# arihantb2/direct_lidar_odometry

Hardware: AMD Instinct MI355X
Metric: gicp_iterations_per_sec (higher is better)
Workload: dtype f64

## Files before the change

direct_lidar_odometry_amd/csrc/ngicp_align.h:

```cpp
#pragma once

namespace {

std::mutex& persist_mutex(int device) {
  static std::mutex m[64];
  return m[(unsigned)device % 64u];
}

route::Facts route_facts(const ngicp* h, route::Caller caller, int nblocks = 1) {
  route::Facts f;
  f.caller = caller;
  f.persist = h->persist;
  f.robust = h->robust_kind != NGICP_ROBUST_NONE;
  f.prior = h->prior_set;
  f.iterating = h->p.max_iter > 0;
  f.nblocks = nblocks;
  f.pass_slots = h->pass_slots;
  f.persist_slots = h->persist_slots;
  f.max_passes = max_passes(h->p);
  return f;
}
void refuse_for(const ngicp* h, route::Entry e) {
  const std::string why = route::entry_refusal(e, h->voxel_res > 0.0, h->robust_kind != NGICP_ROBUST_NONE, h->prior_set);
  if (!why.empty()) throw ArgError{NGICP_ERR_ARG, why};
}
void refuse_route(const ngicp* h, route::Caller caller, const char* entry) {
  const std::string why = route::refusal(route::switches(), h->sw, route_facts(h, caller), entry);
  if (!why.empty()) throw ArgError{NGICP_ERR_ARG, why};
}
route::Variant pass_variant(const ngicp* h, route::Caller caller, int nblocks) {
  return route::choose_route(route::switches(), h->sw, route_facts(h, caller, nblocks)).variant;
}
void fill_robust(const ngicp* h, int& kind, double& c, double& c2) {
  kind = h->robust_kind;
  c = h->robust_width;
  c2 = h->robust_width * h->robust_width;
}

void launch_pass(ngicp* h, const PassArgs& a, const route::Variant& v, int nblocks, hipStream_t s, hipEvent_t start = nullptr, hipEvent_t stop = nullptr) {
  using K = void (*)(PassArgs);
  const bool four = v.waves == 4;
  K kernel = nullptr;
  PassArgs b = a;
  unsigned grid = (unsigned)nblocks;
  switch (v.family) {
    case route::Family::Staged: {
      int need = kStGrowMax;
      if (h->p.max_corr_dist < 1e30) need = (int)std::ceil(h->p.max_corr_dist / (double)a.grid.h);
      b.stage_grow = std::max(1, std::min(kStGrowMax, need));
      kernel = four ? K(k_gicp_pass_st<4>) : K(k_gicp_pass_st<3>);
      break;
    }
    case route::Family::Queue:
      grid = (unsigned)std::min(nblocks, h->queue_slots[four]);
      kernel = four ? K(k_gicp_queue<2, 4>) : K(k_gicp_queue<2, 3>);
      break;
    case route::Family::Walks:
      if (v.fused) kernel = four ? K(k_gicp_pass<2, 4, true>) : K(k_gicp_pass<2, 3, true>);
      else if (v.robust) kernel = four ? K(k_gicp_pass<2, 4, false, true>) : K(k_gicp_pass<2, 3, false, true>);
      else kernel = four ? K(k_gicp_pass<2, 4>) : K(k_gicp_pass<2, 3>);
      break;
  }
  hipExtLaunchKernelGGL(kernel, dim3(grid), dim3(256), 0, s, start, stop, 0, b);
}

struct LoopCtx {
  PassArgs pa;
  SolveArgs sa;
  int nblocks;
};

void prepare_loop(ngicp* h, LoopCtx& c, bool own_buffers = true, bool with_target = true) {
  ensure_slot_ready(h, h->src, "source");
  if (with_target) ensure_slot_ready(h, h->tgt, "target");
  if (h->src_covs.n != h->src.dev->n) compute_covs(h, h->src, h->src_covs, "source");
  if (with_target && h->tgt_covs.n != h->tgt.dev->n) compute_covs(h, h->tgt, h->tgt_covs, "target");
  DeviceCloud& S = *h->src.dev;
  const size_t n = S.n;
  const int nblocks = std::max(1, (S.n_batches + 3) / 4);
  const int max_rows = max_trace_rows(h->p);
  if (own_buffers) {
    for (int i = 0; i < 2; ++i) {
      h->tpt[i].ensure(n * sizeof(float4));
      h->mahal[i].ensure(n * 6 * sizeof(double));
    }
    h->partials.ensure((size_t)kNumSlots * nblocks * sizeof(double));
    h->grp_order.ensure((size_t)nblocks * sizeof(int));
    h->grp_order_alt.ensure((size_t)nblocks * sizeof(int));
    h->grp_cost.ensure((size_t)nblocks * sizeof(int));
    {
      const long ring = (long)max_rows + 1;
      h->state.ensure(sizeof(LmState) + (ring <= kMaxPersistPasses ? (size_t)ring * kViewWords * sizeof(int) : 0));
    }
    if (h->trace.ensure_grew((size_t)max_rows * kTraceCols * sizeof(double))) h->trace_rows_dev = 0;
    h->sums.ensure(kPartialStride * sizeof(double));
    h->batch_far.ensure((size_t)S.n_batches + 16);
    h->gen_lines.ensure((size_t)kGenLines * kGenStride * sizeof(int));
  }

  PassArgs& a = c.pa;
  fill_robust(h, a.robust_kind, a.robust_c, a.robust_c2);
  a.qpts = S.qpts.as<float4>();
  a.batches = S.batches.as<int2>();
  a.batch_boxes = S.batch_boxes.as<float>();
  int* const order_buf[2] = {own_buffers ? h->grp_order.as<int>() : nullptr, own_buffers ? h->grp_order_alt.as<int>() : nullptr};
  int* const ctl = own_buffers ? h->order_flag.as<int>() : nullptr;
  int* const order_flag[2] = {ctl, ctl ? ctl + 3 : nullptr};
  a.grp_order = order_buf[h->order_sel];
  a.grp_cost = own_buffers ? h->grp_cost.as<int>() : nullptr;
  a.n_batches = S.n_batches;
  a.cov_src = covs_for(h, h->src_covs, h->src.dev);
  a.n_src = (int)n;
  if (with_target) {
    DeviceCloud& T = *h->tgt.dev;
    a.tgt = T.pts();
    a.tgt3 = T.xyz3();
    a.tgtp = T.xyzp();
    a.tgt_cell_start = T.cells();
    a.tgt_cell_box = (h->sw.cell_boxes && T.has_boxes) ? T.cell_box.as<unsigned int>() + kCellPad : nullptr;
    a.cov_tgt = covs_for(h, h->tgt_covs, h->tgt.dev);
    a.grid = T.grid;
  } else {
    a.tgt = nullptr;
    a.tgt3 = nullptr;
    a.tgtp = nullptr;
    a.tgt_cell_start = nullptr;
    a.tgt_cell_box = nullptr;
    a.cov_tgt = nullptr;
    a.grid = Grid{};
  }
  for (int i = 0; i < 2; ++i) {
    a.tpt[i] = own_buffers ? h->tpt[i].as<float4>() : nullptr;
    a.mahal[i] = own_buffers ? h->mahal[i].as<double>() : nullptr;
  }
  a.gate_sq = h->p.max_corr_dist * h->p.max_corr_dist;
  {
    float f = (float)a.gate_sq;
    if ((double)f < a.gate_sq) f = std::nextafter(f, std::numeric_limits<float>::infinity());
    a.gate_sq_f = f;
  }
  a.batch_far = own_buffers ? h->batch_far.as<unsigned char>() : nullptr;
  a.st = own_buffers ? h->state.as<LmState>() : nullptr;
  a.partials = own_buffers ? h->partials.as<double>() : nullptr;
  a.mode = 3;
  a.dbg_stamps = nullptr;
  a.dbg_qstats = nullptr;
  a.dbg_span = nullptr;
  a.order_valid = order_flag[h->order_sel];
  a.t_first = nullptr;
  a.fused = 0;
  a.persist = 0;
  a.first_pass = 0;
  a.max_passes = 0;
  a.ticket = ctl ? ctl + 1 : nullptr;
  a.gen = own_buffers ? h->gen_lines.as<int>() : nullptr;
  {
    int need = kStageMaxGrow;
    if (with_target && h->p.max_corr_dist < 1e30) need = (int)std::ceil(h->p.max_corr_dist / (double)a.grid.h);
    a.stage_grow = h->sw.stage_grow <= 0 ? 0 : std::max(1, std::min(std::min(kStageMaxGrow, h->sw.stage_grow), need));
  }

  SolveArgs& s = c.sa;
  s.st = a.st;
  s.cfg.max_iterations = h->p.max_iter;
  s.cfg.lm_max_iterations = h->p.lm_max_iter;
  s.cfg.optimizer = h->p.optimizer;
  s.cfg.rot_eps = h->p.rot_eps;
  s.cfg.trans_eps = h->p.trans_eps;
  s.cfg.lm_init_lambda_factor = h->p.lm_init_lambda_factor;
  s.partials = a.partials;
  s.nblocks = nblocks;
  s.grp_order = order_buf[h->order_sel];
  s.grp_cost = a.grp_cost;
  s.trace = own_buffers ? h->trace.as<double>() : nullptr;
  s.max_trace_rows = max_rows;
  s.mode = 0;
  s.sums_out = nullptr;
  s.dbg_stamps = nullptr;
  s.progress_host = nullptr;
  s.final_host = nullptr;
  s.order_valid = order_flag[h->order_sel];
  s.t_first = nullptr;
  s.persist = 0;
  s.pass_honours_word = 0;
  s.serial_step = h->sw.serial_step;
  s.pass_ticks = nullptr;
  s.prior = h->prior_set ? h->prior_dev.as<double>() : nullptr;
  s.st_out = nullptr;
  s.nrows = 0;
  a.crow_in = nullptr;
  a.crow_out = nullptr;
  a.cluster_ticket = nullptr;
  a.done_flag = nullptr;
  c.nblocks = nblocks;
  if (!own_buffers) return;
  h->stats.lanes_per_query = 2;
  h->stats.voxel_size = a.grid.h;
  h->stats.grid_dims[0] = a.grid.nx;
  h->stats.grid_dims[1] = a.grid.ny;
  h->stats.grid_dims[2] = a.grid.nz;
}

void init_state_from_pose(LmState& st, const Pose& x0) {
  std::memset(&st, 0, sizeof(st));
  st.hot.x0 = x0;
  st.hot.xi = x0;
  pose_identity(st.hot.delta);
  for (int r = 0; r < 3; ++r) {
    for (int c = 0; c < 3; ++c) st.xi_f[r * 4 + c] = (float)x0.R[r * 3 + c];
    st.xi_f[r * 4 + 3] = (float)x0.t[r];
  }
  std::memcpy(&st.view[kViewXi], &st.hot.xi, sizeof(Pose));
  std::memcpy(&st.view[kViewXiF], st.xi_f, sizeof(st.xi_f));
  static_assert(sizeof(Pose) == 24 * sizeof(int) && kViewXiF == 24 && sizeof(LmState::xi_f) == 12 * sizeof(int), "LmState::view layout");
  st.hot.lambda = -1.0;
  st.hot.nu = 2.0;
  for (int i = 0; i < 6; ++i) st.hot.final_H[i * 6 + i] = 1.0;
}

template <class F>
Pose pose_from_colmajor(const F m[16]) {
  Pose p;
  for (int r = 0; r < 3; ++r) {
    for (int c = 0; c < 3; ++c) p.R[r * 3 + c] = (double)m[c * 4 + r];
    p.t[r] = (double)m[12 + r];
  }
  return p;
}
void pose_to_colmajor_f(const Pose& p, float m[16]) {
  for (int r = 0; r < 3; ++r) {
    for (int c = 0; c < 3; ++c) m[c * 4 + r] = (float)p.R[r * 3 + c];
    m[12 + r] = (float)p.t[r];
    m[r * 4 + 3] = 0.f;
  }
  m[15] = 1.f;
}

inline void wait_for_the_loop(ngicp* h, unsigned long& spins, double t_loop) {
  if ((++spins & (h->host_wait ? 0xfff : 0xfffff)) == 0 && now_ms() - t_loop > 30000.0) throw ArgError{NGICP_ERR_HIP, "the registration loop did not finish within 30 s"};
  if (h->host_wait) sched_yield(); else __builtin_ia32_pause();
}

void store_result(const LmHot& r, float T[16], int* converged, int* nr_iterations, double* hessian) {
  pose_to_colmajor_f(r.x0, T);
  if (converged) *converged = r.converged;
  if (nr_iterations) *nr_iterations = r.nr_iterations;
  if (hessian)
    for (int rr = 0; rr < 6; ++rr)
      for (int cc = 0; cc < 6; ++cc) hessian[cc * 6 + rr] = r.final_H[rr * 6 + cc];
  if (r.lm_failed) std::fprintf(stderr, "lm not converged!!\n");
}

void publish_alignment(ngicp* h, const LmState& st, float loop_ms, float* aligned, size_t out_stride) {
  store_result(st.hot, h->final_T, &h->converged, &h->nr_iterations, h->final_hessian);
  h->trace_host.clear();
  h->trace_rows_dev = (size_t)st.hot.n_trace;
  if (aligned) download_transformed(h, *h->src.dev, h->final_T, aligned, out_stride);
  if (st.hot.have_lin) h->hook_valid = 2;
  ngicp_stats& s = h->stats;
  s.loop_ms = loop_ms;
  s.passes = st.hot.passes;
  s.outer_iterations = st.hot.nr_iterations + 1;
  s.lm_trials = st.hot.n_trace;
  s.search_passes = st.hot.search_passes;
  s.mean_candidates = st.hot.search_passes > 0 ? st.hot.cand_total / ((double)st.hot.search_passes * (double)h->src.dev->n) : 0.0;
  s.valid_fraction = st.hot.search_passes > 0 ? st.hot.valid_total / ((double)st.hot.search_passes * (double)h->src.dev->n) : 0.0;
  s.pass_ms_total = 0.0;
  s.passes_timed = 0;
}

void sum_event_pass_times(ngicp* h, long passes) {
  if (!h->profiling) return;
  ngicp_stats& s = h->stats;
  const long timed = std::min<long>(passes, (long)h->prof_events.size() / 2);
  int counted = 0;
  for (long i = h->prof_stride / 2; i < timed; i += h->prof_stride) {
    float ms = 0.f;
    if (hipEventElapsedTime(&ms, h->prof_events[2 * i], h->prof_events[2 * i + 1]) == hipSuccess) {
      s.pass_ms_total += ms;
      ++counted;
    }
  }
  s.passes_timed = counted;
}

struct Alignment {
  double t_begin = now_ms(), t_loop = 0.0;
  LmState st;
  float loop_ms = 0.f;
  unsigned long spins = 0;
};

void reset_results(ngicp* h) {
  h->hook_valid = 0;
  h->converged = 0;
  h->nr_iterations = 0;
  std::memcpy(h->final_T, kIdentity16, sizeof(kIdentity16));
}

const LmState& upload_initial_state(ngicp* h, const float guess[16]) {
  LmState& st = h->pin_state[0];
  init_state_from_pose(st, pose_from_colmajor(guess));
  if (h->p.max_iter <= 0) st.hot.done = 1;
  HIP_TRY(hipMemcpyAsync(h->state.p, &st, sizeof(st), hipMemcpyHostToDevice, h->stream));
  return st;
}

void begin_alignment(ngicp* h, Alignment& al, const float guess[16], SolveArgs& sa, unsigned long long*& pass_t_first) {
  al.st = upload_initial_state(h, guess);
  *h->h_progress = 0;
  sa.progress_host = h->h_progress;
  sa.final_host = h->pin_final;
  sa.t_first = h->t_first.as<unsigned long long>();
  pass_t_first = h->t_first.as<unsigned long long>();
  al.t_loop = now_ms();
}

template <class Launch>
void feed_alignment(ngicp* h, Alignment& al, long max_launches, Launch&& launch) {
  if (h->p.max_iter <= 0) {
    HIP_TRY(hipStreamSynchronize(h->stream));
// ... 666 lines not shown
```

direct_lidar_odometry_amd/csrc/ngicp_lm.h:

```cpp
#pragma once
#include <stddef.h>

#include "ngicp_math.h"
#include "ngicp_terms.h"

namespace ngk {

struct LmConfig {
  int max_iterations;
  int lm_max_iterations;
  int optimizer;
  double rot_eps, trans_eps;
  double lm_init_lambda_factor;
};

struct LmHot {
  Pose x0;
  Pose xi;
  Pose delta;
  double H[36];
  double b[6];
  double y0;
  double d[6];
  double lambda, nu;
  double cand_total;
  double valid_total;
  double staged_total;
  int iter;
  int trial;
  int have_lin;
  int cur;
  int done;
  int converged;
  int nr_iterations;
  int lm_failed;
  int n_trace;
  int passes;
  int pending;
  double final_H[36];
  unsigned long long t_first, t_done;
  float lin_f[12];
  int lin_unneeded;
  int search_passes;
};
constexpr int kViewXi = 0;
constexpr int kViewXiF = 24;
constexpr int kViewDone = 36, kViewCur = 37, kViewHaveLin = 38;
struct LmState {
  LmHot hot;
  float xi_f[12];
  alignas(512) int view[128];
};
constexpr int kViewWords = 128;
constexpr int kGenLines = 256, kGenStride = 32;
static_assert(sizeof(LmState) % 512 == 0 && offsetof(LmState, view) % 512 == 0, "ring entries are 512-byte aligned");

struct PassPose {
  double R[9], t[3];
  float Tf[12];
  int have_lin, cur;
};
typedef const LmState __attribute__((address_space(4))) * KernelStatePtr;
template <class S>
__device__ __forceinline__ void load_pose(S st, PassPose& p) {
  p.have_lin = st->hot.have_lin;
  p.cur = st->hot.cur;
#pragma unroll
  for (int i = 0; i < 9; ++i) p.R[i] = st->hot.xi.R[i];
#pragma unroll
  for (int i = 0; i < 3; ++i) p.t[i] = st->hot.xi.t[i];
#pragma unroll
  for (int i = 0; i < 12; ++i) p.Tf[i] = st->xi_f[i];
}

struct SolveArgs {
  LmState* st;
  LmConfig cfg;
  const double* partials;
  int nblocks;
  double* trace;
  int max_trace_rows;
  int mode;
  double* sums_out;
  int* grp_order;
  const int* grp_cost;
  unsigned long long* dbg_stamps;
  int* progress_host;
  LmHot* final_host;
  int* order_valid;
  const unsigned long long* t_first;
  LmState* st_out;
  int nrows;
  int persist;
  int pass_honours_word;
  int serial_step;
  unsigned long long* pass_ticks;
  const double* prior;
};

static_assert(offsetof(SolveArgs, pass_ticks) == offsetof(SolveArgs, pass_honours_word) + 8, "serial_step takes no room of its own");

__host__ __device__ __forceinline__ int tri21(int r, int c) { return r * 6 - (r * (r - 1)) / 2 + (c - r); }

constexpr int kMaxOrderGroups = 4096;
constexpr int kSolveThreads = 512;
constexpr int kSolveRowSubsets = 32;
constexpr int kProgressDone = 1 << 30, kProgressMask = kProgressDone - 1;

__device__ __forceinline__ bool is_converged_dev(const Pose& d, double rot_eps, double trans_eps) {
  double rmax = 0.0, tmax = 0.0;
#pragma unroll
  for (int r = 0; r < 3; ++r) {
#pragma unroll
    for (int c = 0; c < 3; ++c) rmax = fmax(rmax, 1.0 / rot_eps * fabs(d.R[r * 3 + c] - (r == c ? 1.0 : 0.0)));
    tmax = fmax(tmax, 1.0 / trans_eps * fabs(d.t[r]));
  }
  return fmax(rmax, tmax) < 1;
}

__device__ __forceinline__ double lm_gain_den(const double* d, const double* b, const double lambda) {
  double den = 0.0;
#pragma unroll
  for (int i = 0; i < 6; ++i) den += d[i] * (lambda * d[i] - b[i]);
  return den;
}
__device__ __forceinline__ double lm_step_norm2(const double* d) {
  double dn = 0.0;
#pragma unroll
  for (int i = 0; i < 6; ++i) dn += d[i] * d[i];
  return dn;
}
__device__ __forceinline__ double lm_lambda_accepted(const double lambda, const double rho) {
  const double q = 2 * rho - 1;
  return lambda * fmax(1.0 / 3.0, 1 - q * q * q);
}

__device__ __forceinline__ void make_trial(LmHot& L, double lambda_add) {
  double A[36], rhs[6];
#pragma unroll
  for (int i = 0; i < 36; ++i) A[i] = L.H[i];
#pragma unroll
  for (int i = 0; i < 6; ++i) {
    A[i * 6 + i] += lambda_add;
    rhs[i] = -L.b[i];
  }
  ldlt6_solve(A, rhs, L.d);
  pose_identity(L.delta);
  so3_exp_matrix(L.d, L.delta.R);
  L.delta.t[0] = L.d[3];
  L.delta.t[1] = L.d[4];
  L.delta.t[2] = L.d[5];
  pose_mul(L.delta, L.x0, L.xi);
}

__device__ __forceinline__ void set_lin_unneeded(LmHot& L, const LmConfig& cfg) {
  L.lin_unneeded = (is_converged_dev(L.delta, cfg.rot_eps, cfg.trans_eps) || L.iter + 1 >= cfg.max_iterations) ? 1 : 0;
}

__device__ __forceinline__ void adopt_new(LmHot& L, const double* sums) {
#pragma unroll
  for (int r = 0; r < 6; ++r)
#pragma unroll
    for (int c = r; c < 6; ++c) L.H[r * 6 + c] = L.H[c * 6 + r] = sums[tri21(r, c)];
#pragma unroll
  for (int i = 0; i < 6; ++i) L.b[i] = sums[21 + i];
  L.y0 = sums[27];
  L.cur ^= 1;
  L.have_lin = 1;
#pragma unroll
  for (int r = 0; r < 3; ++r) {
#pragma unroll
    for (int c = 0; c < 3; ++c) L.lin_f[r * 4 + c] = (float)L.xi.R[r * 3 + c];
    L.lin_f[r * 4 + 3] = (float)L.xi.t[r];
  }
}

__device__ __forceinline__ bool lm_advance(LmHot& L, const LmConfig& cfg, const double* sums, double* trace, int max_trace_rows) {
  const double yi = sums[28];
  L.passes += 1;
  L.cand_total += sums[29];
  L.valid_total += sums[30];
  L.staged_total += sums[31];

  if (cfg.optimizer == 0) {
    adopt_new(L, sums);
    L.nr_iterations = L.iter;
    make_trial(L, 0.0);
    L.x0 = L.xi;
    L.converged = is_converged_dev(L.delta, cfg.rot_eps, cfg.trans_eps) ? 1 : 0;
    L.iter += 1;
    if (L.converged || L.iter >= cfg.max_iterations) L.done = 1;
    return true;
  }

  if (!L.have_lin) {
    adopt_new(L, sums);
    L.nr_iterations = 0;
    if (L.lambda < 0.0) {
      double m = 0.0;
#pragma unroll
      for (int i = 0; i < 6; ++i) m = fmax(m, fabs(L.H[i * 6 + i]));
      L.lambda = cfg.lm_init_lambda_factor * m;
    }
    L.nu = 2.0;
    L.trial = 0;
    if (cfg.lm_max_iterations <= 0) {
      L.lm_failed = 1;
      L.done = 1;
      return false;
    }
    make_trial(L, L.lambda);
    set_lin_unneeded(L, cfg);
    return false;
  }

  const double den = lm_gain_den(L.d, L.b, L.lambda), dn = lm_step_norm2(L.d);
  const double rho = (L.y0 - yi) / den;
  const bool rejected = rho < 0;
  if (trace && L.n_trace < max_trace_rows) {
    double* row = trace + (size_t)L.n_trace * kTraceCols;
    row[0] = L.iter; row[1] = L.trial; row[2] = L.y0; row[3] = yi;
    row[4] = rho; row[5] = L.lambda; row[6] = sqrt(dn); row[7] = rejected ? 0.0 : 1.0;
    L.n_trace += 1;
  }
  if (rejected) {
    if (is_converged_dev(L.delta, cfg.rot_eps, cfg.trans_eps)) {
      L.converged = 1;
      L.done = 1;
      return false;
    }
    L.lambda = L.nu * L.lambda;
    L.nu = 2 * L.nu;
    L.trial += 1;
    if (L.trial >= cfg.lm_max_iterations) {
      L.lm_failed = 1;
      L.converged = 0;
      L.done = 1;
      return false;
    }
    make_trial(L, L.lambda);
    set_lin_unneeded(L, cfg);
    return false;
  }
  return true;
}

__device__ __forceinline__ void lm_step(LmHot& L, const LmConfig& cfg, const double* sums, double* trace, int max_trace_rows, const bool searched = true) {
  const bool gn = cfg.optimizer == 0;
  L.search_passes += searched ? 1 : 0;
  const bool accepted = lm_advance(L, cfg, sums, trace, max_trace_rows);
  if (accepted) {
#pragma unroll
    for (int i = 0; i < 36; ++i) L.final_H[i] = L.H[i];
    if (!gn) {
      const double rho = (L.y0 - sums[28]) / lm_gain_den(L.d, L.b, L.lambda);
      L.x0 = L.xi;
      L.lambda = lm_lambda_accepted(L.lambda, rho);
      L.converged = is_converged_dev(L.delta, cfg.rot_eps, cfg.trans_eps) ? 1 : 0;
      L.iter += 1;
      if (L.converged || L.iter >= cfg.max_iterations) {
        L.done = 1;
      } else {
        adopt_new(L, sums);
        L.nr_iterations = L.iter;
        L.nu = 2.0;
        L.trial = 0;
        make_trial(L, L.lambda);
        set_lin_unneeded(L, cfg);
      }
    }
  }
  if (gn && !L.done) L.xi = L.x0;
}

__device__ __forceinline__ void wave_sync() {
  __builtin_amdgcn_fence(__ATOMIC_RELEASE, "wavefront");
  __builtin_amdgcn_wave_barrier();
  __builtin_amdgcn_fence(__ATOMIC_ACQUIRE, "wavefront");
}
__device__ __forceinline__ double wave_lane_f64(const double v, const int src_lane) {
  return __hiloint2double(__builtin_amdgcn_readlane(__double2hiint(v), src_lane), __builtin_amdgcn_readlane(__double2loint(v), src_lane));
}
__device__ __forceinline__ double wave_fetch_f64(const double v, const int src_lane) {
  return __hiloint2double(__builtin_amdgcn_ds_bpermute(src_lane << 2, __double2hiint(v)), __builtin_amdgcn_ds_bpermute(src_lane << 2, __double2loint(v)));
}
__device__ __forceinline__ bool wave_agree(const bool b) { return __builtin_amdgcn_readfirstlane(b ? 1 : 0) != 0; }
__device__ __forceinline__ int pose_elem_to_rows(const int e) { return e < 9 ? (e / 3) * 4 + e % 3 : (e - 9) * 4 + 3; }

__device__ __forceinline__ void adopt_new_wave(LmHot& L, const double* sums, const int lane) {
  if (lane < 36) {
    const int i = lane / 6, j = lane - 6 * i;
    L.H[lane] = sums[tri21(min(i, j), max(i, j))];
  }
  if (lane < 6) L.b[lane] = sums[21 + lane];
  if (lane < 12) L.lin_f[pose_elem_to_rows(lane)] = (float)reinterpret_cast<const double*>(&L.xi)[lane];
  if (lane == 0) {
    L.y0 = sums[27];
    L.cur ^= 1;
    L.have_lin = 1;
  }
}

__device__ __forceinline__ void make_trial_wave(LmHot& L, const LmConfig& cfg, const double lambda_add, const bool lin_word, const int iter, const int lane) {
  wave_sync();
  const bool act = lane < 36;
  const int i = act ? lane / 6 : 0, j = act ? lane - 6 * i : 0;
  const int r = max(i, j), c = min(i, j);
  double a = act ? L.H[lane] : 0.0;
  if (act && i == j) a += lambda_add;
  double y[6];
#pragma unroll
  for (int e = 0; e < 6; ++e) y[e] = -L.b[e];
  const bool out_t = lane >= 9;
  const int orow = lane < 12 ? (out_t ? lane - 9 : lane / 3) : 0, ocol = lane < 9 ? lane % 3 : 0;
  double xb[3];
#pragma unroll
  for (int m = 0; m < 3; ++m) xb[m] = out_t ? L.x0.t[m] : L.x0.R[m * 3 + ocol];
  int piv[6];
#pragma unroll
  for (int k = 0; k < 6; ++k) {
    int p = k;
    double best = fabs(wave_lane_f64(a, 7 * k));
#pragma unroll
    for (int q = k + 1; q < 6; ++q) {
      const double v = fabs(wave_lane_f64(a, 7 * q));
      if (v > best) {
        best = v;
        p = q;
      }
    }
    p = __builtin_amdgcn_readfirstlane(p);
    piv[k] = p;
    if (p != k) {
      const int si = i == k ? p : (i == p ? k : i), sj = j == k ? p : (j == p ? k : j);
      a = wave_fetch_f64(a, si * 6 + sj);
    }
    if (k < 5) {
      const double dk = wave_lane_f64(a, 7 * k);
      if (dk != 0.0 && isfinite(dk)) {
        const double scaled = ldlt_scale(a, dk);
        if (act && j == k && i > k) a = scaled;
        const double upd = ldlt_update(wave_fetch_f64(a, r * 6 + c), wave_fetch_f64(a, r * 6 + k), dk, wave_fetch_f64(a, c * 6 + k));
        if (act && i > k && j > k) a = upd;
      }
    }
  }
#pragma unroll
  for (int k = 0; k < 6; ++k)
#pragma unroll
    for (int q = k + 1; q < 6; ++q)
      if (piv[k] == q) {
        const double t = y[k];
        y[k] = y[q];
        y[q] = t;
      }
  double lo[15];
#pragma unroll
  for (int q = 1; q < 6; ++q)
#pragma unroll
    for (int e = 0; e < q; ++e) lo[q * (q - 1) / 2 + e] = wave_lane_f64(a, q * 6 + e);
#pragma unroll
  for (int q = 0; q < 6; ++q)
#pragma unroll
    for (int e = 0; e < q; ++e) y[q] = ldlt_subst(y[q], lo[q * (q - 1) / 2 + e], y[e]);
  {
    double mine = y[0];
#pragma unroll
    for (int q = 1; q < 6; ++q) mine = lane == 7 * q ? y[q] : mine;
    const double dv = ldlt_diag(mine, a);
#pragma unroll
    for (int q = 0; q < 6; ++q) y[q] = wave_lane_f64(dv, 7 * q);
  }
#pragma unroll
  for (int q = 5; q >= 0; --q)
#pragma unroll
    for (int e = q + 1; e < 6; ++e) y[q] = ldlt_subst(y[q], lo[e * (e - 1) / 2 + q], y[e]);
#pragma unroll
  for (int k = 5; k >= 0; --k)
#pragma unroll
    for (int q = k + 1; q < 6; ++q)
      if (piv[k] == q) {
        const double t = y[k];
        y[k] = y[q];
        y[q] = t;
      }
  Pose delta;
  so3_exp_matrix(y, delta.R);
  delta.t[0] = y[3];
  delta.t[1] = y[4];
  delta.t[2] = y[5];
  double ar[3];
#pragma unroll
  for (int m = 0; m < 3; ++m) ar[m] = orow == 0 ? delta.R[m] : (orow == 1 ? delta.R[3 + m] : delta.R[6 + m]);
  const double at = orow == 0 ? delta.t[0] : (orow == 1 ? delta.t[1] : delta.t[2]);
  const double xr = pose_mul_r(ar[0], ar[1], ar[2], xb[0], xb[1], xb[2]), xt = pose_mul_t(ar[0], ar[1], ar[2], xb[0], xb[1], xb[2], at);
  if (lane < 12) reinterpret_cast<double*>(&L.xi)[lane] = out_t ? xt : xr;
  const bool conv = lin_word ? is_converged_dev(delta, cfg.rot_eps, cfg.trans_eps) : false;
  if (lane == 0) {
#pragma unroll
    for (int e = 0; e < 6; ++e) L.d[e] = y[e];
    L.delta = delta;
    if (lin_word) L.lin_unneeded = (conv || iter + 1 >= cfg.max_iterations) ? 1 : 0;
  }
}

__device__ __forceinline__ void lm_step_wave(LmHot& L, const LmConfig& cfg, const double* sums, double* trace, int max_trace_rows, const bool searched, const int lane) {
  const double yi = sums[28];
  int iter = L.iter;
  double lambda = L.lambda;
  const int have_lin = L.have_lin;
  if (lane == 0) {
    L.search_passes += searched ? 1 : 0;
    L.passes += 1;
    L.cand_total += sums[29];
    L.valid_total += sums[30];
    L.staged_total += sums[31];
  }
  const bool gn = cfg.optimizer == 0;
  bool go_on = true;
  if (gn) {
    adopt_new_wave(L, sums, lane);
    lambda = 0.0;
  } else if (!wave_agree(have_lin != 0)) {
    adopt_new_wave(L, sums, lane);
    if (wave_agree(lambda < 0.0)) {
      double m = 0.0;
#pragma unroll
      for (int i = 0; i < 6; ++i) m = fmax(m, fabs(sums[tri21(i, i)]));
      lambda = cfg.lm_init_lambda_factor * m;
    }
    go_on = cfg.lm_max_iterations > 0;
    if (lane == 0) {
      L.nr_iterations = 0;
      L.lambda = lambda;
      L.nu = 2.0;
      L.trial = 0;
      if (!go_on) L.lm_failed = 1, L.done = 1;
    }
  } else {
    double d[6], b[6];
#pragma unroll
    for (int e = 0; e < 6; ++e) d[e] = L.d[e], b[e] = L.b[e];
    const double y0 = L.y0, nu = L.nu;
    const int trial = L.trial, n_trace = L.n_trace;
    const double rho = (y0 - yi) / lm_gain_den(d, b, lambda);
    const bool rejected = wave_agree(rho < 0);
    if (trace && n_trace < max_trace_rows && lane == 0) {
      double* row = trace + (size_t)n_trace * kTraceCols;
      row[0] = iter; row[1] = trial; row[2] = y0; row[3] = yi;
      row[4] = rho; row[5] = lambda; row[6] = sqrt(lm_step_norm2(d)); row[7] = rejected ? 0.0 : 1.0;
      L.n_trace = n_trace + 1;
    }
    const bool conv = wave_agree(is_converged_dev(L.delta, cfg.rot_eps, cfg.trans_eps));
    if (rejected) {
      const bool failed = !conv && trial + 1 >= cfg.lm_max_iterations;
      go_on = !conv && !failed;
      if (!conv) lambda = nu * lambda;
      if (lane == 0) {
        if (conv) {
          L.converged = 1, L.done = 1;
        } else {
          L.lambda = lambda;
          L.nu = 2 * nu;
          L.trial = trial + 1;
          if (failed) L.lm_failed = 1, L.converged = 0, L.done = 1;
        }
      }
    } else {
      if (lane < 36) L.final_H[lane] = L.H[lane];
      if (lane < 12) reinterpret_cast<double*>(&L.x0)[lane] = reinterpret_cast<const double*>(&L.xi)[lane];
      lambda = lm_lambda_accepted(lambda, rho);
      iter += 1;
      go_on = !(conv || iter >= cfg.max_iterations);
      if (lane == 0) {
        L.lambda = lambda;
        L.converged = conv ? 1 : 0;
        L.iter = iter;
        if (!go_on) L.done = 1;
      }
      if (go_on) {
        adopt_new_wave(L, sums, lane);
        if (lane == 0) {
          L.nr_iterations = iter;
          L.nu = 2.0;
          L.trial = 0;
        }
      }
    }
  }
  if (!wave_agree(go_on)) return;
  make_trial_wave(L, cfg, lambda, !gn, iter, lane);
  if (gn) {
    wave_sync();
    if (lane < 12) reinterpret_cast<double*>(&L.x0)[lane] = reinterpret_cast<const double*>(&L.xi)[lane];
    if (lane < 36) L.final_H[lane] = L.H[lane];
    const bool conv = wave_agree(is_converged_dev(L.delta, cfg.rot_eps, cfg.trans_eps));
    if (lane == 0) {
      L.nr_iterations = iter;
      L.converged = conv ? 1 : 0;
      L.iter = iter + 1;
      if (conv || iter + 1 >= cfg.max_iterations) L.done = 1;
    }
  }
}

}
```

direct_lidar_odometry_amd/csrc/ngicp_solve.h:

```cpp
#pragma once
#include "ngicp_lm.h"

namespace ngk {

constexpr int kSolveSubs = kSolveThreads / 16;
#ifndef NGICP_SOLVE_CHUNK
#define NGICP_SOLVE_CHUNK 40
#endif
constexpr int kSolveChunk = NGICP_SOLVE_CHUNK;


template <int THREADS>
struct SolveShared {
  double wsum[32][kPartialStride];
  double sums[kPartialStride];
  int ord_cnt[THREADS / 64 - 1][16], ord_pos[THREADS / 64 - 1][16];
  int ord_cost[kMaxOrderGroups];
  unsigned char ord_cls[kMaxOrderGroups];
  int ord_arrived;
  LmHot L;
};

template <int THREADS>
__device__ __forceinline__ void build_launch_order(const SolveArgs& a, SolveShared<THREADS>& sh, const int lane, const int wave) {
  auto& ord_cnt = sh.ord_cnt;
  auto& ord_pos = sh.ord_pos;
  auto& ord_cost = sh.ord_cost;
  auto& ord_cls = sh.ord_cls;
  int& ord_arrived = sh.ord_arrived;
  const unsigned long long t_ord = a.dbg_stamps ? __builtin_amdgcn_s_memtime() : 0ull;
  constexpr int kSortWaves = THREADS / 64 - 1;
  const int sw = wave - 1;
  auto wsync = [] {
    __builtin_amdgcn_fence(__ATOMIC_RELEASE, "wavefront");
    __builtin_amdgcn_wave_barrier();
    __builtin_amdgcn_fence(__ATOMIC_ACQUIRE, "wavefront");
  };
  auto same_class = [&](int cls, bool valid) -> unsigned long long {
    unsigned long long m = __ballot(valid);
#pragma unroll
    for (int bit = 0; bit < 4; ++bit) {
      const bool one = (cls >> bit) & 1;
      const unsigned long long bb = __ballot(valid && one);
      m &= one ? bb : ~bb;
    }
    return m;
  };
  if (lane < 16) ord_cnt[sw][lane] = 0;
  int mx = 1;
  for (int gi = lane; gi < a.nblocks; gi += 64) mx = max(mx, ord_cost[gi]);
#pragma unroll
  for (int o = 32; o > 0; o >>= 1) mx = max(mx, __shfl_xor(mx, o));
  const float to_class = 16.0f / ((float)mx + 1.0f);
  const unsigned long long lt = (1ull << lane) - 1ull;
  const int slice = ((a.nblocks + kSortWaves * 64 - 1) / (kSortWaves * 64)) * 64;
  const int g_first = sw * slice, g_last = min(g_first + slice, a.nblocks);
  wsync();
  for (int g0 = g_first; g0 < g_last; g0 += 64) {
    const int gi = g0 + lane;
    const bool valid = gi < g_last;
    const int cls = valid ? 15 - min(15, (int)((float)ord_cost[gi] * to_class)) : 0;
    if (valid) ord_cls[gi] = (unsigned char)cls;
    const unsigned long long m = same_class(cls, valid);
    if (valid && (m & lt) == 0) ord_cnt[sw][cls] += __popcll(m);
    wsync();
  }
  __builtin_amdgcn_fence(__ATOMIC_RELEASE, "workgroup");
  if (lane == 0) atomicAdd(&ord_arrived, 1);
  bool met = false;
  for (int spin = 0; spin < (1 << 20); ++spin) {
    if (*reinterpret_cast<volatile int*>(&ord_arrived) >= kSortWaves) {
      met = true;
      break;
    }
    __builtin_amdgcn_s_sleep(2);
  }
  __builtin_amdgcn_fence(__ATOMIC_ACQUIRE, "workgroup");
  if (met) {
    if (lane < 16) {
      int run = 0;
      for (int c = 0; c < lane; ++c)
        for (int w = 0; w < kSortWaves; ++w) run += ord_cnt[w][c];
      for (int w = 0; w < sw; ++w) run += ord_cnt[w][lane];
      ord_pos[sw][lane] = run;
    }
    wsync();
    for (int g0 = g_first; g0 < g_last; g0 += 64) {
      const int gi = g0 + lane;
      const bool valid = gi < g_last;
      const int cls = valid ? ord_cls[gi] : 0;
      const unsigned long long m = same_class(cls, valid);
      const int base = ord_pos[sw][cls];
      if (valid) a.grp_order[base + __popcll(m & lt)] = gi;
      wsync();
      if (valid && (m & lt) == 0) ord_pos[sw][cls] = base + __popcll(m);
      wsync();
    }
    if (sw == 0 && lane == 0 && a.order_valid) *a.order_valid = 1;
  }
  if (a.dbg_stamps && sw == 0 && lane == 0) a.dbg_stamps[7] = __builtin_amdgcn_s_memtime() - t_ord;
}

template <int THREADS, bool AGENT, bool PERSIST = false>
__device__ __forceinline__ void lm_solve_body(const SolveArgs& a, SolveShared<THREADS>& sh) {
  static_assert(!PERSIST || AGENT, "the persistent solver is an agent-scope one");
  constexpr int kSolveThreads = THREADS;
  constexpr int kSolveSubs = 32;
  constexpr int kThreadSubs = THREADS / 16;
  constexpr int kPer = kSolveSubs / kThreadSubs;
  constexpr int kSolveChunk = THREADS >= 512 ? NGICP_SOLVE_CHUNK : 14;
  static_assert(kPer >= 1 && kPer * kThreadSubs == kSolveSubs, "block sizes: 256 or 512 threads");
  auto& wsum = sh.wsum;
  auto& sums = sh.sums;
  auto& ord_cost = sh.ord_cost;
  int& ord_arrived = sh.ord_arrived;
  LmHot& L = sh.L;
  if (threadIdx.x == 0) ord_arrived = 0;
  LmState* st = a.st;
  LmState* sto = a.st_out ? a.st_out : a.st;
#define NG_SSTAMP(k)                                                                 \
  do {                                                                               \
    if (a.dbg_stamps && threadIdx.x == 0) a.dbg_stamps[k] = __builtin_amdgcn_s_memtime(); \
  } while (0)
  const int done_at_entry = PERSIST ? 0 : __hip_atomic_load(&st->hot.done, __ATOMIC_RELAXED, __HIP_MEMORY_SCOPE_WORKGROUP);
  const unsigned long long t_solver_entry = a.dbg_stamps ? __builtin_amdgcn_s_memtime() : 0ull;
  const int lane = threadIdx.x & 63, wave = threadIdx.x >> 6;
  const int vp = threadIdx.x & 15, sb = threadIdx.x >> 4;
  const double2* __restrict__ rows = reinterpret_cast<const double2*>(a.partials) + vp;
  static_assert(sizeof(LmHot) % 4 == 0, "LmHot is copied as dwords");
  constexpr int kHotWords = (int)(sizeof(LmHot) / 4), kHotPerThread = (kHotWords + kSolveThreads - 1) / kSolveThreads;
  constexpr int kCostPerThread = kMaxOrderGroups / kSolveThreads;
  const int passes_at_entry = PERSIST ? __hip_atomic_load(&st->hot.passes, __ATOMIC_RELAXED, __HIP_MEMORY_SCOPE_AGENT) : st->hot.passes;
  const int k4_only_at_entry = (!PERSIST && a.pass_honours_word) ? st->hot.lin_unneeded : 0;
  const bool order_it = a.mode == 0 && a.grp_order && a.nblocks <= kMaxOrderGroups && !k4_only_at_entry && (PERSIST ? passes_at_entry == 2 : (!AGENT || passes_at_entry < 3 || (passes_at_entry & 3) == 3));
  int hv[kHotPerThread];
#pragma unroll
  for (int k = 0; k < kHotPerThread; ++k) {
    const int w = threadIdx.x + k * kSolveThreads;
    if constexpr (PERSIST) hv[k] = w < kHotWords ? __hip_atomic_load(reinterpret_cast<const int*>(&st->hot) + w, __ATOMIC_RELAXED, __HIP_MEMORY_SCOPE_AGENT) : 0;
    else hv[k] = w < kHotWords ? reinterpret_cast<const int*>(&st->hot)[w] : 0;
  }
  const int last_row = (a.nrows ? a.nrows : a.nblocks) - 1, last_grp = a.nblocks - 1;
  auto load_row = [](const double2* q) -> double2 {
    if constexpr (PERSIST) {
      const double* d = reinterpret_cast<const double*>(q);
      return make_double2(__hip_atomic_load(d, __ATOMIC_RELAXED, __HIP_MEMORY_SCOPE_AGENT), __hip_atomic_load(d + 1, __ATOMIC_RELAXED, __HIP_MEMORY_SCOPE_AGENT));
    } else {
      return *q;
    }
  };
  double2 p[kPer * kSolveChunk];
#pragma unroll
  for (int sI = 0; sI < kPer; ++sI)
#pragma unroll
    for (int j = 0; j < kSolveChunk; ++j) {
      const int gi = sb + sI * kThreadSubs + j * kSolveSubs;
      p[sI * kSolveChunk + j] = gi <= last_row ? load_row(rows + (size_t)gi * (kNumSlots / 2)) : make_double2(0.0, 0.0);
    }
  int oc[kCostPerThread];
#pragma unroll
  for (int k = 0; k < kCostPerThread; ++k) {
    const int gi = threadIdx.x + k * kSolveThreads;
    if constexpr (PERSIST) oc[k] = (order_it && gi <= last_grp) ? __hip_atomic_load(a.grp_cost + gi, __ATOMIC_RELAXED, __HIP_MEMORY_SCOPE_AGENT) : 0;
    else oc[k] = (order_it && gi <= last_grp) ? a.grp_cost[gi] : 0;
  }
  double prior_v = 0.0;
  if (a.prior && threadIdx.x < kPriorDoubles) prior_v = a.prior[threadIdx.x];
  if (a.mode == 0 && done_at_entry) return;
  if (a.dbg_stamps && threadIdx.x == 0) a.dbg_stamps[0] = t_solver_entry;
#pragma unroll
  for (int k = 0; k < kHotPerThread; ++k) {
    const int w = threadIdx.x + k * kSolveThreads;
    if (w < kHotWords) reinterpret_cast<int*>(&L)[w] = hv[k];
  }
  if (order_it) {
#pragma unroll
    for (int k = 0; k < kCostPerThread; ++k) {
      const int gi = threadIdx.x + k * kSolveThreads;
      if (gi < a.nblocks) ord_cost[gi] = oc[k];
    }
  }
  {
    double a0[kPer], a1[kPer];
#pragma unroll
    for (int sI = 0; sI < kPer; ++sI) {
      a0[sI] = p[sI * kSolveChunk].x;
      a1[sI] = p[sI * kSolveChunk].y;
#pragma unroll
      for (int j = 1; j < kSolveChunk; ++j) {
        a0[sI] += p[sI * kSolveChunk + j].x;
        a1[sI] += p[sI * kSolveChunk + j].y;
      }
    }
    for (int g0 = kSolveSubs * kSolveChunk; g0 + sb <= last_row; g0 += kSolveSubs * kSolveChunk) {
#pragma unroll
      for (int sI = 0; sI < kPer; ++sI)
#pragma unroll
        for (int j = 0; j < kSolveChunk; ++j) {
          const int gi = g0 + sb + sI * kThreadSubs + j * kSolveSubs;
          p[sI * kSolveChunk + j] = gi <= last_row ? load_row(rows + (size_t)gi * (kNumSlots / 2)) : make_double2(0.0, 0.0);
        }
#pragma unroll
      for (int sI = 0; sI < kPer; ++sI)
#pragma unroll
        for (int j = 0; j < kSolveChunk; ++j) {
          a0[sI] += p[sI * kSolveChunk + j].x;
          a1[sI] += p[sI * kSolveChunk + j].y;
        }
    }
    NG_SSTAMP(1);
#pragma unroll
    for (int sI = 0; sI < kPer; ++sI) {
      wsum[sb + sI * kThreadSubs][2 * vp] = a0[sI];
      wsum[sb + sI * kThreadSubs][2 * vp + 1] = a1[sI];
    }
  }
  __syncthreads();
  if (threadIdx.x < kPartialStride) {
    const int v = threadIdx.x;
    double t = 0.0;
    if (v < kNumSlots)
      for (int sb = 0; sb < kSolveSubs; ++sb) t += wsum[sb][v];
    sums[v] = t;
  }
  __syncthreads();
  NG_SSTAMP(2);
  if (a.sums_out && threadIdx.x < kPartialStride) a.sums_out[threadIdx.x] = sums[threadIdx.x];
  if (a.mode == 3) return;
  if (order_it && wave >= 1) build_launch_order<THREADS>(a, sh, lane, wave);
  if (wave != 0) return;
  if (a.prior) {
    double* const P = &wsum[0][0];
    if (lane < kPriorDoubles) P[lane] = prior_v;
    wave_sync();
    double r[6], theta_sq, jc;
    prior_residual(L.xi, P, r, theta_sq, jc);
    if (lane < 36) P[kPriorDoubles + lane] = prior_jac_elem(lane / 6, lane % 6, r[0], r[1], r[2], theta_sq, jc, L.xi.t[0], L.xi.t[1], L.xi.t[2]);
#pragma unroll
    for (int q = 0; q < 6; ++q)
      if (lane == 36 + q) P[kPriorDoubles + 36 + q] = r[q];
    wave_sync();
    if (lane < kPriorRowSums + 1) sums[lane] += prior_row_elem(lane < kPriorRowSums ? lane : kPriorRowSums - 1, P + kPriorDoubles, P + 12, P + kPriorDoubles + 36);
    wave_sync();
  }
  if (a.mode == 2) {
    if (lane == 0) st->hot.y0 = sums[28];
    return;
  }
  if (a.mode != 1 && !a.serial_step) {
    NG_SSTAMP(3);
    lm_step_wave(L, a.cfg, sums, a.trace, a.max_trace_rows, !(a.pass_honours_word && L.lin_unneeded), lane);
    NG_SSTAMP(4);
    wave_sync();
    NG_SSTAMP(5);
    if (!L.done && lane < 12) {
      const float f = (float)reinterpret_cast<const double*>(&L.xi)[lane];
      if constexpr (PERSIST) __hip_atomic_store(&st->xi_f[pose_elem_to_rows(lane)], f, __ATOMIC_RELAXED, __HIP_MEMORY_SCOPE_AGENT);
      else sto->xi_f[pose_elem_to_rows(lane)] = f;
    }
  } else if (lane == 0) {
    if (a.mode == 1) {
      adopt_new(L, sums);
    } else {
      const LmConfig& cfg = a.cfg;
      NG_SSTAMP(3);
      lm_step(L, cfg, sums, a.trace, a.max_trace_rows, !(a.pass_honours_word && L.lin_unneeded));
      NG_SSTAMP(4);
      NG_SSTAMP(5);
      if (!L.done) {
#pragma unroll
        for (int r = 0; r < 3; ++r) {
#pragma unroll
          for (int c = 0; c < 4; ++c) {
            const float f = (float)(c < 3 ? L.xi.R[r * 3 + c] : L.xi.t[r]);
            if constexpr (PERSIST) __hip_atomic_store(&st->xi_f[r * 4 + c], f, __ATOMIC_RELAXED, __HIP_MEMORY_SCOPE_AGENT);
            else sto->xi_f[r * 4 + c] = f;
          }
        }
      }
    }
  }
  if (a.mode == 0 && lane == 0 && L.done) {
    L.t_done = __builtin_amdgcn_s_memrealtime();
    if (a.t_first) L.t_first = PERSIST ? __hip_atomic_load(a.t_first, __ATOMIC_RELAXED, __HIP_MEMORY_SCOPE_AGENT) : *a.t_first;
  }
  __builtin_amdgcn_fence(__ATOMIC_RELEASE, "wavefront");
  __builtin_amdgcn_wave_barrier();
  __builtin_amdgcn_fence(__ATOMIC_ACQUIRE, "wavefront");
  const bool finished_now = a.mode == 0 && L.done != 0;
  if constexpr (!PERSIST) {
    for (int w = lane; w < (int)(sizeof(LmHot) / 4); w += 64) reinterpret_cast<int*>(&sto->hot)[w] = reinterpret_cast<const int*>(&L)[w];
  }
  if (finished_now && a.final_host) {
    for (int w = lane; w < (int)(sizeof(LmHot) / 4); w += 64)
      __hip_atomic_store(reinterpret_cast<int*>(a.final_host) + w, reinterpret_cast<const int*>(&L)[w], __ATOMIC_RELAXED, __HIP_MEMORY_SCOPE_SYSTEM);
    __threadfence_system();
    __builtin_amdgcn_wave_barrier();
  }
  if (a.mode == 0 && a.progress_host && lane == 0)
    __hip_atomic_store(a.progress_host, (L.passes & kProgressMask) | (L.done ? kProgressDone : 0), __ATOMIC_RELAXED, __HIP_MEMORY_SCOPE_SYSTEM);
  if constexpr (PERSIST) {
    for (int w = lane; w < (int)(sizeof(LmHot) / 4); w += 64)
      __hip_atomic_store(reinterpret_cast<int*>(&st->hot) + w, reinterpret_cast<const int*>(&L)[w], __ATOMIC_RELAXED, __HIP_MEMORY_SCOPE_AGENT);
    int v = 0;
    if (lane < 24) {
      v = reinterpret_cast<const int*>(&L.xi)[lane];
    } else if (lane < 36) {
      const int r = (lane - 24) >> 2, cI = (lane - 24) & 3;
      v = __float_as_int((float)(cI < 3 ? L.xi.R[r * 3 + cI] : L.xi.t[r]));
    } else if (lane == kViewDone) {
      v = L.done;
    } else if (lane == kViewCur) {
      v = L.cur;
    } else if (lane == kViewHaveLin) {
      v = L.have_lin;
    }
    __hip_atomic_store(st->view + (size_t)L.passes * kViewWords + lane, v, __ATOMIC_RELAXED, __HIP_MEMORY_SCOPE_AGENT);
  }
  NG_SSTAMP(6);
#undef NG_SSTAMP
}

__global__ void __launch_bounds__(kSolveThreads) k_lm_solve(SolveArgs a) {
  __shared__ SolveShared<kSolveThreads> sh;
  lm_solve_body<kSolveThreads, false>(a, sh);
}

constexpr int kStepSelftestIn = 132;
constexpr size_t kStepSelftestRecord = sizeof(LmHot) + 18 * sizeof(double);
static_assert(sizeof(LmHot) % 8 == 0, "the trace row behind the image is 8-byte aligned");
__global__ void __launch_bounds__(64) k_step_selftest(const double* __restrict__ in, int n_problems, unsigned char* __restrict__ out) {
  __shared__ LmHot L;
  __shared__ double sums[kPartialStride];
  static_assert(kPartialStride >= 32, "32 reduced sums");
  const int lane = threadIdx.x;
  if ((int)blockIdx.x >= n_problems) return;
  const double* p = in + (size_t)blockIdx.x * kStepSelftestIn;
  LmConfig cfg;
  cfg.max_iterations = (int)p[93];
  cfg.lm_max_iterations = (int)p[94];
  cfg.optimizer = (int)p[95];
  cfg.rot_eps = p[96];
  cfg.trans_eps = p[97];
  cfg.lm_init_lambda_factor = p[98];
  const bool searched = p[131] != 0.0;
  for (int form = 0; form < 2; ++form) {
    unsigned char* rec = out + ((size_t)blockIdx.x * 2 + form) * kStepSelftestRecord;
    double* tail = reinterpret_cast<double*>(rec + sizeof(LmHot));
    __syncthreads();
    for (int w = lane; w < (int)(sizeof(LmHot) / 4); w += 64) reinterpret_cast<int*>(&L)[w] = 0;
    if (lane < 32) sums[lane] = p[99 + lane];
    __syncthreads();
    if (lane < 36) reinterpret_cast<double*>(&L.x0)[lane] = p[lane];
    if (lane < 36) L.H[lane] = p[36 + lane];
    if (lane < 6) L.b[lane] = p[72 + lane], L.d[lane] = p[79 + lane];
    if (lane == 0) {
      L.y0 = p[78];
      L.lambda = p[85];
      L.nu = p[86];
      L.iter = (int)p[87];
      L.trial = (int)p[88];
      L.have_lin = (int)p[89];
      L.cur = (int)p[90];
      L.n_trace = max(0, (int)p[91]);
      L.lin_unneeded = (int)p[92];
    }
    __syncthreads();
    if (form == 0) {
      if (lane == 0) lm_step(L, cfg, sums, tail, 1, searched);
    } else {
      lm_step_wave(L, cfg, sums, tail, 1, searched, lane);
    }
    __syncthreads();
    for (int w = lane; w < (int)(sizeof(LmHot) / 4); w += 64) reinterpret_cast<int*>(rec)[w] = reinterpret_cast<const int*>(&L)[w];
    if (lane < 6) tail[8 + lane] = L.d[lane];
    if (lane == 0) tail[14] = L.done, tail[15] = L.converged, tail[16] = L.lm_failed, tail[17] = L.trial;
  }
}
static_assert(offsetof(LmHot, xi) == offsetof(LmHot, x0) + sizeof(Pose) && offsetof(LmHot, delta) == offsetof(LmHot, xi) + sizeof(Pose), "x0, xi, delta are contiguous");

}
```

Baseline: 21000.

## Cache trial convergence, precompute inverse epsilons, vectorize state copy, relax sync

Stores the reciprocal rotation and translation tolerances in the LM config so the convergence test multiplies instead of divides. It caches the convergence verdict of each trial step in a new LmHot field, so the accept and reject paths reuse it instead of recomputing it. The non-persistent state write-back now uses 16-byte stores, and one block-wide barrier after the sums reduction becomes a wave-level sync. The wave sync is only safe if a single wave reads the reduced sums; otherwise it opens a race.

```diff
diff --git a/direct_lidar_odometry_amd/csrc/ngicp_align.h b/direct_lidar_odometry_amd/csrc/ngicp_align.h
--- a/direct_lidar_odometry_amd/csrc/ngicp_align.h
+++ b/direct_lidar_odometry_amd/csrc/ngicp_align.h
@@ -165,8 +165,7 @@
   s.cfg.max_iterations = h->p.max_iter;
   s.cfg.lm_max_iterations = h->p.lm_max_iter;
   s.cfg.optimizer = h->p.optimizer;
-  s.cfg.rot_eps = h->p.rot_eps;
-  s.cfg.trans_eps = h->p.trans_eps;
+  lm_config_set_eps(s.cfg, h->p.rot_eps, h->p.trans_eps);
   s.cfg.lm_init_lambda_factor = h->p.lm_init_lambda_factor;
   s.partials = a.partials;
   s.nblocks = nblocks;
diff --git a/direct_lidar_odometry_amd/csrc/ngicp_lm.h b/direct_lidar_odometry_amd/csrc/ngicp_lm.h
--- a/direct_lidar_odometry_amd/csrc/ngicp_lm.h
+++ b/direct_lidar_odometry_amd/csrc/ngicp_lm.h
@@ -10,9 +10,13 @@
   int max_iterations;
   int lm_max_iterations;
   int optimizer;
-  double rot_eps, trans_eps;
+  double inv_rot_eps, inv_trans_eps;
   double lm_init_lambda_factor;
 };
+__host__ __device__ __forceinline__ void lm_config_set_eps(LmConfig& c, double rot_eps, double trans_eps) {
+  c.inv_rot_eps = 1.0 / rot_eps;
+  c.inv_trans_eps = 1.0 / trans_eps;
+}
 
 struct LmHot {
   Pose x0;
@@ -37,12 +41,17 @@
   int n_trace;
   int passes;
   int pending;
+  int trial_converged;
   double final_H[36];
   unsigned long long t_first, t_done;
   float lin_f[12];
   int lin_unneeded;
   int search_passes;
 };
+static_assert(offsetof(LmHot, trial_converged) + 4 == offsetof(LmHot, final_H) && sizeof(LmHot) % 8 == 0, "trial_converged fills what was padding: no field moved");
+static_assert(offsetof(LmHot, iter) == 720 && offsetof(LmHot, trial) == 724 && offsetof(LmHot, done) == 736 && offsetof(LmHot, converged) == 740 &&
+              offsetof(LmHot, lm_failed) == 748 && offsetof(LmHot, trial_converged) == 764 && offsetof(LmHot, lin_unneeded) == 1120 && offsetof(LmHot, delta) == 192,
+              "the offsets the step tests read");
 constexpr int kViewXi = 0;
 constexpr int kViewXiF = 24;
 constexpr int kViewDone = 36, kViewCur = 37, kViewHaveLin = 38;
@@ -107,13 +116,13 @@
 constexpr int kSolveRowSubsets = 32;
 constexpr int kProgressDone = 1 << 30, kProgressMask = kProgressDone - 1;
 
-__device__ __forceinline__ bool is_converged_dev(const Pose& d, double rot_eps, double trans_eps) {
+__device__ __forceinline__ bool is_converged_dev(const Pose& d, double inv_rot_eps, double inv_trans_eps) {
   double rmax = 0.0, tmax = 0.0;
 #pragma unroll
   for (int r = 0; r < 3; ++r) {
 #pragma unroll
-    for (int c = 0; c < 3; ++c) rmax = fmax(rmax, 1.0 / rot_eps * fabs(d.R[r * 3 + c] - (r == c ? 1.0 : 0.0)));
-    tmax = fmax(tmax, 1.0 / trans_eps * fabs(d.t[r]));
+    for (int c = 0; c < 3; ++c) rmax = fmax(rmax, inv_rot_eps * fabs(d.R[r * 3 + c] - (r == c ? 1.0 : 0.0)));
+    tmax = fmax(tmax, inv_trans_eps * fabs(d.t[r]));
   }
   return fmax(rmax, tmax) < 1;
 }
@@ -154,7 +163,9 @@
 }
 
 __device__ __forceinline__ void set_lin_unneeded(LmHot& L, const LmConfig& cfg) {
-  L.lin_unneeded = (is_converged_dev(L.delta, cfg.rot_eps, cfg.trans_eps) || L.iter + 1 >= cfg.max_iterations) ? 1 : 0;
+  const bool conv = is_converged_dev(L.delta, cfg.inv_rot_eps, cfg.inv_trans_eps);
+  L.trial_converged = conv ? 1 : 0;
+  L.lin_unneeded = (conv || L.iter + 1 >= cfg.max_iterations) ? 1 : 0;
 }
 
 __device__ __forceinline__ void adopt_new(LmHot& L, const double* sums) {
@@ -187,7 +198,7 @@
     L.nr_iterations = L.iter;
     make_trial(L, 0.0);
     L.x0 = L.xi;
-    L.converged = is_converged_dev(L.delta, cfg.rot_eps, cfg.trans_eps) ? 1 : 0;
+    L.converged = is_converged_dev(L.delta, cfg.inv_rot_eps, cfg.inv_trans_eps) ? 1 : 0;
     L.iter += 1;
     if (L.converged || L.iter >= cfg.max_iterations) L.done = 1;
     return true;
@@ -224,7 +235,7 @@
     L.n_trace += 1;
   }
   if (rejected) {
-    if (is_converged_dev(L.delta, cfg.rot_eps, cfg.trans_eps)) {
+    if (L.trial_converged) {
       L.converged = 1;
       L.done = 1;
       return false;
@@ -256,7 +267,7 @@
       const double rho = (L.y0 - sums[28]) / lm_gain_den(L.d, L.b, L.lambda);
       L.x0 = L.xi;
       L.lambda = lm_lambda_accepted(L.lambda, rho);
-      L.converged = is_converged_dev(L.delta, cfg.rot_eps, cfg.trans_eps) ? 1 : 0;
+      L.converged = L.trial_converged ? 1 : 0;
       L.iter += 1;
       if (L.converged || L.iter >= cfg.max_iterations) {
         L.done = 1;
@@ -395,12 +406,12 @@
   const double at = orow == 0 ? delta.t[0] : (orow == 1 ? delta.t[1] : delta.t[2]);
   const double xr = pose_mul_r(ar[0], ar[1], ar[2], xb[0], xb[1], xb[2]), xt = pose_mul_t(ar[0], ar[1], ar[2], xb[0], xb[1], xb[2], at);
   if (lane < 12) reinterpret_cast<double*>(&L.xi)[lane] = out_t ? xt : xr;
-  const bool conv = lin_word ? is_converged_dev(delta, cfg.rot_eps, cfg.trans_eps) : false;
+  const bool conv = lin_word ? is_converged_dev(delta, cfg.inv_rot_eps, cfg.inv_trans_eps) : false;
   if (lane == 0) {
 #pragma unroll
     for (int e = 0; e < 6; ++e) L.d[e] = y[e];
     L.delta = delta;
-    if (lin_word) L.lin_unneeded = (conv || iter + 1 >= cfg.max_iterations) ? 1 : 0;
+    if (lin_word) L.trial_converged = conv ? 1 : 0, L.lin_unneeded = (conv || iter + 1 >= cfg.max_iterations) ? 1 : 0;
   }
 }
 
@@ -451,7 +462,7 @@
       row[4] = rho; row[5] = lambda; row[6] = sqrt(lm_step_norm2(d)); row[7] = rejected ? 0.0 : 1.0;
       L.n_trace = n_trace + 1;
     }
-    const bool conv = wave_agree(is_converged_dev(L.delta, cfg.rot_eps, cfg.trans_eps));
+    const bool conv = wave_agree(L.trial_converged != 0);
     if (rejected) {
       const bool failed = !conv && trial + 1 >= cfg.lm_max_iterations;
       go_on = !conv && !failed;
@@ -494,7 +505,7 @@
     wave_sync();
     if (lane < 12) reinterpret_cast<double*>(&L.x0)[lane] = reinterpret_cast<const double*>(&L.xi)[lane];
     if (lane < 36) L.final_H[lane] = L.H[lane];
-    const bool conv = wave_agree(is_converged_dev(L.delta, cfg.rot_eps, cfg.trans_eps));
+    const bool conv = wave_agree(is_converged_dev(L.delta, cfg.inv_rot_eps, cfg.inv_trans_eps));
     if (lane == 0) {
       L.nr_iterations = iter;
       L.converged = conv ? 1 : 0;
diff --git a/direct_lidar_odometry_amd/csrc/ngicp_solve.h b/direct_lidar_odometry_amd/csrc/ngicp_solve.h
--- a/direct_lidar_odometry_amd/csrc/ngicp_solve.h
+++ b/direct_lidar_odometry_amd/csrc/ngicp_solve.h
@@ -18,7 +18,7 @@
   int ord_cost[kMaxOrderGroups];
   unsigned char ord_cls[kMaxOrderGroups];
   int ord_arrived;
-  LmHot L;
+  alignas(16) LmHot L;
 };
 
 template <int THREADS>
@@ -223,7 +223,7 @@
       for (int sb = 0; sb < kSolveSubs; ++sb) t += wsum[sb][v];
     sums[v] = t;
   }
-  __syncthreads();
+  wave_sync();
   NG_SSTAMP(2);
   if (a.sums_out && threadIdx.x < kPartialStride) a.sums_out[threadIdx.x] = sums[threadIdx.x];
   if (a.mode == 3) return;
@@ -289,7 +289,10 @@
   __builtin_amdgcn_fence(__ATOMIC_ACQUIRE, "wavefront");
   const bool finished_now = a.mode == 0 && L.done != 0;
   if constexpr (!PERSIST) {
-    for (int w = lane; w < (int)(sizeof(LmHot) / 4); w += 64) reinterpret_cast<int*>(&sto->hot)[w] = reinterpret_cast<const int*>(&L)[w];
+    constexpr int kHot16 = (int)(sizeof(LmHot) / 16);
+    static_assert(sizeof(LmHot) % 16 == 8 && offsetof(LmState, hot) == 0 && alignof(LmState) >= 16, "70 sixteen-byte words and one of eight");
+    for (int w = lane; w < kHot16; w += 64) reinterpret_cast<int4*>(&sto->hot)[w] = reinterpret_cast<const int4*>(&L)[w];
+    if (lane == kHot16 % 64) reinterpret_cast<int2*>(&sto->hot)[2 * kHot16] = reinterpret_cast<const int2*>(&L)[2 * kHot16];
   }
   if (finished_now && a.final_host) {
     for (int w = lane; w < (int)(sizeof(LmHot) / 4); w += 64)
@@ -330,7 +333,7 @@
 constexpr size_t kStepSelftestRecord = sizeof(LmHot) + 18 * sizeof(double);
 static_assert(sizeof(LmHot) % 8 == 0, "the trace row behind the image is 8-byte aligned");
 __global__ void __launch_bounds__(64) k_step_selftest(const double* __restrict__ in, int n_problems, unsigned char* __restrict__ out) {
-  __shared__ LmHot L;
+  __shared__ alignas(16) LmHot L;
   __shared__ double sums[kPartialStride];
   static_assert(kPartialStride >= 32, "32 reduced sums");
   const int lane = threadIdx.x;
@@ -340,8 +343,7 @@
   cfg.max_iterations = (int)p[93];
   cfg.lm_max_iterations = (int)p[94];
   cfg.optimizer = (int)p[95];
-  cfg.rot_eps = p[96];
-  cfg.trans_eps = p[97];
+  lm_config_set_eps(cfg, p[96], p[97]);
   cfg.lm_init_lambda_factor = p[98];
   const bool searched = p[131] != 0.0;
   for (int form = 0; form < 2; ++form) {
@@ -364,6 +366,9 @@
       L.cur = (int)p[90];
       L.n_trace = max(0, (int)p[91]);
       L.lin_unneeded = (int)p[92];
+      Pose delta;
+      for (int e = 0; e < 12; ++e) reinterpret_cast<double*>(&delta)[e] = p[24 + e];
+      L.trial_converged = is_converged_dev(delta, cfg.inv_rot_eps, cfg.inv_trans_eps) ? 1 : 0;
     }
     __syncthreads();
     if (form == 0) {
```

Measured after the change: 21180 (median of 6 runs). About the same (+0.9%).
